# GradientSpaces/LivingScenes

Measured on AMD Instinct MI355X. Metric: object-instances/sec (encode+match+register), N=1024 pts, higher is better.
Workload: dtype f32 (GEMM products as two-piece f16 splits on the f16 matrix cores, fp32 accumulate: as accurate against fp64 as an fp32 FMA chain)

## Files before the change

### livingscenes_amd/csrc/edge_fused.hip

```cpp
#include "ls_common.h"

namespace ls {

constexpr int FK = 16;
constexpr int FND = 32;
typedef _Float16 fh8_t __attribute__((ext_vector_type(8)));
typedef _Float16 fh2_t __attribute__((ext_vector_type(2)));
typedef float ff2_t __attribute__((ext_vector_type(2)));
typedef float ff16_t __attribute__((ext_vector_type(16)));

__device__ __forceinline__ void fsplit_pair(ff2_t v, unsigned& h, unsigned& l) {
    const fh2_t hv = __builtin_convertvector(v, fh2_t);
    const fh2_t lv = __builtin_convertvector(v - __builtin_convertvector(hv, ff2_t), fh2_t);
    h = __builtin_bit_cast(unsigned, hv);
    l = __builtin_bit_cast(unsigned, lv);
}
__device__ __forceinline__ void fpow2(float amax, float& s, int& e_inv) {
    unsigned be = (__float_as_uint(amax) >> 23) & 0xffu;
    be = be < 15u ? 15u : be;
    s = __uint_as_float((268u - be) << 23);
    e_inv = (int)be - 14 - 127;
}
template <int CTRL>
__device__ __forceinline__ float fdpp_max(float v) {
    return fmaxf(v, __int_as_float(__builtin_amdgcn_update_dpp(__float_as_int(v), __float_as_int(v), CTRL, 0xF, 0xF, false)));
}
template <int CTRL>
__device__ __forceinline__ float fdpp_add(float v) {
    return v + __int_as_float(__builtin_amdgcn_update_dpp(0, __float_as_int(v), CTRL, 0xF, 0xF, true));
}
__device__ __forceinline__ float fquad_sum(float v) { return fdpp_add<0x4E>(fdpp_add<0xB1>(v)); }
__device__ __forceinline__ float fquad_max(float v) { return fdpp_max<0x4E>(fdpp_max<0xB1>(v)); }
__device__ __forceinline__ float finv_fro(float ss) { return __builtin_amdgcn_rsqf(fmaxf(ss, 1e-24f)); }

__global__ __launch_bounds__(64) void edge_ft_presplit_w_kernel(const float* __restrict__ W, int Co, int Cin, int KS, uint4* __restrict__ planes,
                                                                int* __restrict__ wexp) {
    const int T = blockIdx.x / KS, ks = blockIdx.x % KS, lane = threadIdx.x;
    const int head = T / 5, p = T % 5, r = lane & 31;
    const float* wr = W + ((size_t)(2 * p + (r >> 4)) * Co + 16 * head + (r & 15)) * Cin;
    float am = 0.f;
    for (int c = 0; c < Cin; ++c) am = fmaxf(am, fabsf(wr[c]));
    float sc;
    int e;
    fpow2(am, sc, e);
    if (ks == 0 && lane < 32) wexp[T * 32 + r] = e;
    const int k = ks * 16 + 8 * (lane >> 5);
    uint4 h, l;
    fsplit_pair(ff2_t{wr[k] * sc, wr[k + 1] * sc}, h.x, l.x);
    fsplit_pair(ff2_t{wr[k + 2] * sc, wr[k + 3] * sc}, h.y, l.y);
    fsplit_pair(ff2_t{wr[k + 4] * sc, wr[k + 5] * sc}, h.z, l.z);
    fsplit_pair(ff2_t{wr[k + 6] * sc, wr[k + 7] * sc}, h.w, l.w);
    planes[((size_t)blockIdx.x * 2) * 64 + lane] = h;
    planes[((size_t)blockIdx.x * 2 + 1) * 64 + lane] = l;
}
size_t edge_ft_w_bytes(int Co, int Cin) { return (size_t)(Co / 16) * 5 * (Cin / 16) * 2 * 64 * sizeof(uint4) + (size_t)(Co / 16) * 5 * 32 * sizeof(int); }
int edge_ft_presplit_w_launch(const float* W, int Co, int Cin, void* planes, hipStream_t st) {
    const int tiles = (Co / 16) * 5, KS = Cin / 16;
    hipLaunchKernelGGL(edge_ft_presplit_w_kernel, dim3(tiles * KS), dim3(64), 0, st, W, Co, Cin, KS, (uint4*)planes,
                       (int*)((uint4*)planes + (size_t)tiles * KS * 128));
    LS_LAUNCH_CHECK();
    return LS_OK;
}

template <int KS>
__global__ __launch_bounds__(256) void edge_ft_prep_a_kernel(const float* __restrict__ cur, const int32_t* __restrict__ rows, int Ns, int Nd,
                                                             uint4* __restrict__ planes, int* __restrict__ aexp) {
    constexpr int CIN = KS * 16, KPW = KS / 4;
    __shared__ float lmax[4][32];
    const int lane = threadIdx.x & 63, w = threadIdx.x >> 6, j = lane & 31, h = lane >> 5;
    const int R = blockIdx.x * 32 + j;
    size_t src = (size_t)R;
    if (rows) {
        const int x = R % 3, pn = R / 3, b = pn / Nd;
        src = ((size_t)b * Ns + rows[pn]) * 3 + x;
    }
    const float* rp = cur + src * CIN + (w * KPW) * 16 + h * 8;
    float4 v[KPW][2];
    float am = 0.f;
#pragma unroll
    for (int kk = 0; kk < KPW; ++kk) {
        v[kk][0] = *reinterpret_cast<const float4*>(rp + kk * 16);
        v[kk][1] = *reinterpret_cast<const float4*>(rp + kk * 16 + 4);
    }
#pragma unroll
    for (int kk = 0; kk < KPW; ++kk)
#pragma unroll
        for (int u = 0; u < 2; ++u)
            am = fmaxf(am, fmaxf(fmaxf(fabsf(v[kk][u].x), fabsf(v[kk][u].y)), fmaxf(fabsf(v[kk][u].z), fabsf(v[kk][u].w))));
    am = fmaxf(am, __shfl_xor(am, 32, 64));
    if (h == 0) lmax[w][j] = am;
    __syncthreads();
    am = fmaxf(fmaxf(lmax[0][j], lmax[1][j]), fmaxf(lmax[2][j], lmax[3][j]));
    float sc;
    int e;
    fpow2(am, sc, e);
    if (w == 0 && h == 0) aexp[R] = e;
#pragma unroll
    for (int kk = 0; kk < KPW; ++kk) {
        uint4 hh, ll;
        fsplit_pair(ff2_t{v[kk][0].x * sc, v[kk][0].y * sc}, hh.x, ll.x);
        fsplit_pair(ff2_t{v[kk][0].z * sc, v[kk][0].w * sc}, hh.y, ll.y);
        fsplit_pair(ff2_t{v[kk][1].x * sc, v[kk][1].y * sc}, hh.z, ll.z);
        fsplit_pair(ff2_t{v[kk][1].z * sc, v[kk][1].w * sc}, hh.w, ll.w);
        uint4* op = planes + (((size_t)blockIdx.x * KS + w * KPW + kk) * 2) * 64 + lane;
        op[0] = hh;
        op[64] = ll;
    }
}

struct FT43 { float4 x, y, z; };
__device__ __forceinline__ FT43 ft_lds43(const float* p, int sld) {
    FT43 r;
    r.x = *reinterpret_cast<const float4*>(p);
    r.y = *reinterpret_cast<const float4*>(p + sld);
    r.z = *reinterpret_cast<const float4*>(p + 2 * sld);
    return r;
}
__device__ __forceinline__ FT43 ft_add43(const FT43& a, const FT43& b) {
    FT43 r;
    r.x = make_float4(a.x.x + b.x.x, a.x.y + b.x.y, a.x.z + b.x.z, a.x.w + b.x.w);
    r.y = make_float4(a.y.x + b.y.x, a.y.y + b.y.y, a.y.z + b.y.z, a.y.w + b.y.w);
    r.z = make_float4(a.z.x + b.z.x, a.z.y + b.z.y, a.z.z + b.z.z, a.z.w + b.z.w);
    return r;
}
__device__ __forceinline__ void ft_act43(FT43& y, const FT43& k, float oms) {
    vn_act(y.x.x, y.y.x, y.z.x, k.x.x, k.y.x, k.z.x, oms);
    vn_act(y.x.y, y.y.y, y.z.y, k.x.y, k.y.y, k.z.y, oms);
    vn_act(y.x.z, y.y.z, y.z.z, k.x.z, k.y.z, k.z.z, oms);
    vn_act(y.x.w, y.y.w, y.z.w, k.x.w, k.y.w, k.z.w, oms);
}
__device__ __forceinline__ float ft_dot43(const FT43& a, const FT43& b) {
    float s = a.x.x * b.x.x;
    s = __builtin_fmaf(a.y.x, b.y.x, s); s = __builtin_fmaf(a.z.x, b.z.x, s);
    s = __builtin_fmaf(a.x.y, b.x.y, s); s = __builtin_fmaf(a.y.y, b.y.y, s); s = __builtin_fmaf(a.z.y, b.z.y, s);
    s = __builtin_fmaf(a.x.z, b.x.z, s); s = __builtin_fmaf(a.y.z, b.y.z, s); s = __builtin_fmaf(a.z.z, b.z.z, s);
    s = __builtin_fmaf(a.x.w, b.x.w, s); s = __builtin_fmaf(a.y.w, b.y.w, s); s = __builtin_fmaf(a.z.w, b.z.w, s);
    return s;
}
__device__ __forceinline__ void ft_fma43(FT43& acc, float w, const FT43& y) {
    acc.x.x = __builtin_fmaf(w, y.x.x, acc.x.x); acc.x.y = __builtin_fmaf(w, y.x.y, acc.x.y); acc.x.z = __builtin_fmaf(w, y.x.z, acc.x.z); acc.x.w = __builtin_fmaf(w, y.x.w, acc.x.w);
    acc.y.x = __builtin_fmaf(w, y.y.x, acc.y.x); acc.y.y = __builtin_fmaf(w, y.y.y, acc.y.y); acc.y.z = __builtin_fmaf(w, y.y.z, acc.y.z); acc.y.w = __builtin_fmaf(w, y.y.w, acc.y.w);
    acc.z.x = __builtin_fmaf(w, y.z.x, acc.z.x); acc.z.y = __builtin_fmaf(w, y.z.y, acc.z.y); acc.z.z = __builtin_fmaf(w, y.z.z, acc.z.z); acc.z.w = __builtin_fmaf(w, y.z.w, acc.z.w);
}

template <int KS>
struct FtJob { const uint4* a_planes; const int* a_exp; int mt0; int MT; int p; float* slab; int sld; };

template <int KS, int MPU>
__device__ __forceinline__ void ft_gemm_unit(const FtJob<KS>& jb, int tile0, int hl, int T, const uint4* __restrict__ wplanes, const int* __restrict__ wexp, int lane) {
    const char* ab = reinterpret_cast<const char*>(jb.a_planes + ((size_t)(jb.mt0 + tile0) * KS * 2) * 64);
    const char* wb = reinterpret_cast<const char*>(wplanes + ((size_t)T * KS * 2) * 64);
    const int we = wexp[T * 32 + (lane & 31)];
    ff16_t acc[MPU];
#pragma unroll
    for (int m = 0; m < MPU; ++m)
#pragma unroll
        for (int r = 0; r < 16; ++r) acc[m][r] = 0.f;
    unsigned voff = (unsigned)lane * 16u;
    constexpr int KB = 2;
    struct Stage { fh8_t ah[MPU][KB], al[MPU][KB], bh[KB], bl[KB]; };
    auto load_stage = [&](Stage& sg, int k0) {
        asm volatile("" : "+v"(voff));
#pragma unroll
        for (int u = 0; u < KB; ++u) {
            sg.bh[u] = __builtin_bit_cast(fh8_t, *reinterpret_cast<const uint4*>(wb + (size_t)((k0 + u) * 2) * 1024 + voff));
            sg.bl[u] = __builtin_bit_cast(fh8_t, *reinterpret_cast<const uint4*>(wb + (size_t)((k0 + u) * 2 + 1) * 1024 + voff));
#pragma unroll
            for (int m = 0; m < MPU; ++m) {
                sg.ah[m][u] = __builtin_bit_cast(fh8_t, *reinterpret_cast<const uint4*>(ab + (size_t)((m * KS + k0 + u) * 2) * 1024 + voff));
                sg.al[m][u] = __builtin_bit_cast(fh8_t, *reinterpret_cast<const uint4*>(ab + (size_t)((m * KS + k0 + u) * 2 + 1) * 1024 + voff));
            }
        }
    };
    auto run_stage = [&](const Stage& sg) {
#pragma unroll
        for (int u = 0; u < KB; ++u)
#pragma unroll
            for (int m = 0; m < MPU; ++m) {
                acc[m] = __builtin_amdgcn_mfma_f32_32x32x16_f16(sg.al[m][u], sg.bh[u], acc[m], 0, 0, 0);
                acc[m] = __builtin_amdgcn_mfma_f32_32x32x16_f16(sg.ah[m][u], sg.bh[u], acc[m], 0, 0, 0);
                acc[m] = __builtin_amdgcn_mfma_f32_32x32x16_f16(sg.ah[m][u], sg.bl[u], acc[m], 0, 0, 0);
            }
#pragma unroll
        for (int m = 0; m < MPU; ++m) asm volatile("" : "+v"(acc[m])::"memory");
    };
#pragma unroll
    for (int k0 = 0; k0 < KS; k0 += KB) {
        Stage sg;
        load_stage(sg, k0);
        __builtin_amdgcn_sched_barrier(0);
        run_stage(sg);
    }
#pragma unroll
    for (int m = 0; m < MPU; ++m) {
        const int mt = tile0 + m;
        const int row0 = 32 * mt + 4 * (lane >> 5);
        float* sp = jb.slab + (size_t)row0 * jb.sld + hl * 32 + (lane & 31);
        const int* ae = jb.a_exp + (jb.mt0 + mt) * 32 + 4 * (lane >> 5);
#pragma unroll
        for (int r = 0; r < 16; ++r) {
            const int dr = (r & 3) + 8 * (r >> 2);
            sp[dr * jb.sld] = __builtin_ldexpf(acc[m][r], ae[dr] + we);
        }
    }
}
template <int KS, int HG, int NJ>
__device__ __forceinline__ void ft_gemm_phase_g3(const FtJob<KS> (&jobs)[NJ], const uint4* __restrict__ wplanes, const int* __restrict__ wexp, int head0,
                                                 int wave, int lane) {
    if constexpr (NJ == 2 && HG == 1) {
        if (jobs[0].MT == 12 && jobs[1].MT == 3) {
            ft_gemm_unit<KS, 3>(jobs[0], 3 * wave, 0, head0 * 5 + jobs[0].p, wplanes, wexp, lane);
            if (wave < 3) ft_gemm_unit<KS, 1>(jobs[1], wave, 0, head0 * 5 + jobs[1].p, wplanes, wexp, lane);
            return;
        }
    }
    int total = 0;
#pragma unroll
    for (int j = 0; j < NJ; ++j) total += (jobs[j].MT / 3) * HG;
    for (int t = wave; t < total; t += 4) {
        int j = 0, off = t;
#pragma unroll
        for (int q = 0; q < NJ - 1; ++q)
            if (j == q && off >= (jobs[q].MT / 3) * HG) { off -= (jobs[q].MT / 3) * HG; j = q + 1; }
        FtJob<KS> jb = jobs[0];
#pragma unroll
        for (int q = 1; q < NJ; ++q)
            if (j == q) jb = jobs[q];
        const int ng = jb.MT / 3, hl = off / ng, g = off - hl * ng;
        ft_gemm_unit<KS, 3>(jb, 3 * g, hl, (head0 + hl) * 5 + jb.p, wplanes, wexp, lane);
    }
}

template <int KS, int HG, int NJ>
__device__ __forceinline__ void ft_gemm_phase_shared(const FtJob<KS> (&jobs)[NJ], const uint4* __restrict__ wplanes, const int* __restrict__ wexp, int head0,
                                                     int wave, int lane, uint4* ring) {
    const bool has_unit = wave < NJ * HG;
    const int j = has_unit ? wave / HG : 0, hl = wave % HG;
    FtJob<KS> jb = jobs[0];
#pragma unroll
    for (int q = 1; q < NJ; ++q)
        if (j == q) jb = jobs[q];
    const int T = (head0 + hl) * 5 + jb.p;
    const char* ab = reinterpret_cast<const char*>(jobs[0].a_planes + ((size_t)jobs[0].mt0 * KS * 2) * 64);
    const char* wb = reinterpret_cast<const char*>(wplanes + ((size_t)T * KS * 2) * 64);
    const int we = wexp[T * 32 + (lane & 31)];
    ff16_t acc[3];
#pragma unroll
    for (int m = 0; m < 3; ++m)
#pragma unroll
        for (int r = 0; r < 16; ++r) acc[m][r] = 0.f;
    unsigned voff = (unsigned)lane * 16u;
    auto a_addr = [&](int k0, int f) { const int u = f / 6, m = (f % 6) / 2, pl = f % 2; return ab + (size_t)((m * KS + k0 + u) * 2 + pl) * 1024 + voff; };
    constexpr int NB = KS / 2;
    uint4 sA_r0, sA_r1, sA_r2, sA_w0, sA_w1, sA_w2, sA_w3, sB_r0, sB_r1, sB_r2, sB_w0, sB_w1, sB_w2, sB_w3, sC_r0, sC_r1, sC_r2, sC_w0, sC_w1, sC_w2, sC_w3;
#define LS_FT_LOAD_BATCH(S, K0)                                                                           \
    {                                                                                                     \
        asm volatile("" : "+v"(voff));                                                                    \
        S##_r0 = *reinterpret_cast<const uint4*>(a_addr((K0), wave * 3 + 0));                             \
        S##_r1 = *reinterpret_cast<const uint4*>(a_addr((K0), wave * 3 + 1));                             \
        S##_r2 = *reinterpret_cast<const uint4*>(a_addr((K0), wave * 3 + 2));                             \
        S##_w0 = *reinterpret_cast<const uint4*>(wb + (size_t)(((K0) + 0) * 2) * 1024 + voff);            \
        S##_w1 = *reinterpret_cast<const uint4*>(wb + (size_t)(((K0) + 0) * 2 + 1) * 1024 + voff);        \
        S##_w2 = *reinterpret_cast<const uint4*>(wb + (size_t)(((K0) + 1) * 2) * 1024 + voff);            \
        S##_w3 = *reinterpret_cast<const uint4*>(wb + (size_t)(((K0) + 1) * 2 + 1) * 1024 + voff);        \
    }
#define LS_FT_STEP(S, BI)                                                                                                                          \
    {                                                                                                                                              \
        uint4* rb = ring + ((BI) & 1) * 12 * 64;                                                                                                   \
        rb[(wave * 3 + 0) * 64 + lane] = S##_r0;                                                                                                   \
        rb[(wave * 3 + 1) * 64 + lane] = S##_r1;                                                                                                   \
        rb[(wave * 3 + 2) * 64 + lane] = S##_r2;                                                                                                   \
        const fh8_t bh0 = __builtin_bit_cast(fh8_t, S##_w0), bl0 = __builtin_bit_cast(fh8_t, S##_w1), bh1 = __builtin_bit_cast(fh8_t, S##_w2),     \
                    bl1 = __builtin_bit_cast(fh8_t, S##_w3);                                                                                       \
        if ((BI) + 3 < NB) LS_FT_LOAD_BATCH(S, 2 * ((BI) + 3))                                                                                     \
        __syncthreads();                                                                                                                           \
        if (has_unit) {                                                                                                                            \
            _Pragma("unroll") for (int u = 0; u < 2; ++u) {                                                                                        \
                const fh8_t bh = u ? bh1 : bh0, bl = u ? bl1 : bl0;                                                                                \
                _Pragma("unroll") for (int m = 0; m < 3; ++m) {                                                                                    \
                    const fh8_t ah = __builtin_bit_cast(fh8_t, rb[(u * 6 + m * 2) * 64 + lane]), al = __builtin_bit_cast(fh8_t, rb[(u * 6 + m * 2 + 1) * 64 + lane]); \
                    acc[m] = __builtin_amdgcn_mfma_f32_32x32x16_f16(al, bh, acc[m], 0, 0, 0);                                                      \
                    acc[m] = __builtin_amdgcn_mfma_f32_32x32x16_f16(ah, bh, acc[m], 0, 0, 0);                                                      \
                    acc[m] = __builtin_amdgcn_mfma_f32_32x32x16_f16(ah, bl, acc[m], 0, 0, 0);                                                      \
                }                                                                                                                                  \
            }                                                                                                                                      \
        }                                                                                                                                          \
    }
    LS_FT_LOAD_BATCH(sA, 0)
    if (1 < NB) LS_FT_LOAD_BATCH(sB, 2)
    if (2 < NB) LS_FT_LOAD_BATCH(sC, 4)
#pragma unroll
    for (int bi = 0; bi < NB; bi += 3) {
        LS_FT_STEP(sA, bi)
        if (bi + 1 < NB) LS_FT_STEP(sB, bi + 1)
        if (bi + 2 < NB) LS_FT_STEP(sC, bi + 2)
    }
#undef LS_FT_STEP
#undef LS_FT_LOAD_BATCH
    if (has_unit) {
#pragma unroll
        for (int m = 0; m < 3; ++m) {
            const int row0 = 32 * m + 4 * (lane >> 5);
            float* sp = jb.slab + (size_t)row0 * jb.sld + hl * 32 + (lane & 31);
            const int* ae = jb.a_exp + (jb.mt0 + m) * 32 + 4 * (lane >> 5);
#pragma unroll
            for (int r = 0; r < 16; ++r) {
                const int dr = (r & 3) + 8 * (r >> 2);
                sp[dr * jb.sld] = __builtin_ldexpf(acc[m][r], ae[dr] + we);
            }
        }
    }
}

template <int HG>
struct FtMap {
    int n, hl, ql, k0, kn;
    __device__ __forceinline__ FtMap(int tid) {
        ql = tid & 3;
        const int idx = tid >> 2;
        n = idx >> 1;
        if constexpr (HG == 2) { hl = idx & 1; k0 = 0; kn = FK; }
        else { hl = 0; k0 = (idx & 1) * (FK / 2); kn = FK / 2; }
    }
};

template <int CIN, int NS, int HG>
__global__ __launch_bounds__(256, 2) void edge_ft_qk_kernel(const uint4* __restrict__ a_p, const int* __restrict__ ae_p, const uint4* __restrict__ a_q,
                                                         const int* __restrict__ ae_q, const uint4* __restrict__ wplanes, const int* __restrict__ wexp,
                                                         const int32_t* __restrict__ knn, int B, int H, float oms, float* __restrict__ scores,
                                                         float* __restrict__ sskp, float* __restrict__ ssqp) {
    constexpr int KS = CIN / 16, MTP = NS * 3 / 32, MTQ = FND * 3 / 32, SLD = HG * 32 + 4;
    __shared__ __attribute__((aligned(16))) float slab_q[FND * 3 * SLD];
    __shared__ __attribute__((aligned(16))) float slab_p[NS * 3 * SLD];
    __shared__ __attribute__((aligned(16))) uint4 a_ring[NS == 32 ? 2 * 12 * 64 : 1];
    const int tid = threadIdx.x, lane = tid & 63, wave = __builtin_amdgcn_readfirstlane(tid >> 6);
    const int logical = xcd_remap(blockIdx.x, gridDim.x);
    const int ngroups = H / HG;
    const int hg = logical % ngroups, b = logical / ngroups, head0 = hg * HG;
    const FtMap<HG> mp(tid);
    const int head = head0 + mp.hl;

    {
        const FtJob<KS> jq[1] = {{a_q, ae_q, b * MTQ, MTQ, 4, slab_q, SLD}};
        if constexpr (NS == 32) ft_gemm_phase_shared<KS, HG, 1>(jq, wplanes, wexp, head0, wave, lane, a_ring);
        else ft_gemm_phase_g3<KS, HG, 1>(jq, wplanes, wexp, head0, wave, lane);
    }
    __syncthreads();
    const int c4 = mp.hl * 32 + mp.ql * 4;
    FT43 qf = ft_lds43(slab_q + (size_t)(3 * mp.n) * SLD + c4, SLD);
    {
        const FT43 kd = ft_lds43(slab_q + (size_t)(3 * mp.n) * SLD + c4 + 16, SLD);
        ft_act43(qf, kd, oms);
    }
    const float ssq = fquad_sum(ft_dot43(qf, qf));
    if (mp.ql == 0 && mp.k0 == 0) ssqp[((size_t)b * H + head) * FND + mp.n] = ssq;
    int nb[FK];
    {
        const int4* kp = reinterpret_cast<const int4*>(knn + ((size_t)b * FND + mp.n) * FK + mp.k0);
#pragma unroll
        for (int u = 0; u < FK / 4; ++u)
            if (4 * u < mp.kn) { const int4 v = kp[u]; nb[4 * u] = v.x; nb[4 * u + 1] = v.y; nb[4 * u + 2] = v.z; nb[4 * u + 3] = v.w; }
    }
    __syncthreads();

    {
        const FtJob<KS> jk[2] = {{a_p, ae_p, b * MTP, MTP, 1, slab_p, SLD}, {a_q, ae_q, b * MTQ, MTQ, 3, slab_q, SLD}};
        if constexpr (NS == 32) ft_gemm_phase_shared<KS, HG, 2>(jk, wplanes, wexp, head0, wave, lane, a_ring);
        else ft_gemm_phase_g3<KS, HG, 2>(jk, wplanes, wexp, head0, wave, lane);
    }
    __syncthreads();
    {
        const FT43 ql = ft_lds43(slab_q + (size_t)(3 * mp.n) * SLD + c4, SLD), qd = ft_lds43(slab_q + (size_t)(3 * mp.n) * SLD + c4 + 16, SLD);
        float* so = scores + (((size_t)b * H + head) * FND + mp.n) * FK + mp.k0;
        float* ko = sskp + (((size_t)b * H + head) * FND + mp.n) * FK + mp.k0;
#pragma unroll
        for (int k = 0; k < FK; ++k) {
            if (k < mp.kn) {
                const float* pr = slab_p + (size_t)(3 * nb[k]) * SLD + c4;
                FT43 y = ft_add43(ft_lds43(pr, SLD), ql);
                const FT43 kd = ft_add43(ft_lds43(pr + 16, SLD), qd);
                ft_act43(y, kd, oms);
                const float s2 = fquad_sum(ft_dot43(y, y));
                const float a = fquad_sum(ft_dot43(y, qf));
                if (mp.ql == 0) { so[k] = a; ko[k] = s2; }
            }
        }
    }
}

__global__ __launch_bounds__(256) void edge_ft_norms_kernel(const float* __restrict__ sskp, const float* __restrict__ ssqp, int H, float* __restrict__ invk,
                                                            float* __restrict__ invq) {
    LS_LATENCY_CRITICAL();
    const int b = blockIdx.x, tid = threadIdx.x;
    for (int e = tid; e < FND * FK + FND; e += 256) {
        const bool isk = e < FND * FK;
        const int stride = isk ? FND * FK : FND;
        const float* sp = isk ? sskp + (size_t)b * H * FND * FK + e : ssqp + (size_t)b * H * FND + (e - FND * FK);
        float s = 0.f;
        int h = 0;
        for (; h + 8 <= H; h += 8) {
            float v[8];
#pragma unroll
            for (int u = 0; u < 8; ++u) v[u] = sp[(size_t)(h + u) * stride];
#pragma unroll
            for (int u = 0; u < 8; ++u) s += v[u];
        }
        for (; h < H; ++h) s += sp[(size_t)h * stride];
        if (isk) invk[(size_t)b * FND * FK + e] = finv_fro(s);
        else invq[(size_t)b * FND + (e - FND * FK)] = finv_fro(s);
    }
}

template <int CIN, int NS, int HG>
__global__ __launch_bounds__(256, 2) void edge_ft_v_kernel(const uint4* __restrict__ a_p, const int* __restrict__ ae_p, const uint4* __restrict__ a_q,
                                                        const int* __restrict__ ae_q, const uint4* __restrict__ wplanes, const int* __restrict__ wexp,
                                                        const int32_t* __restrict__ knn, int B, int H, float oms, float inv_sqrt_dk,
                                                        const float* __restrict__ scores, const float* __restrict__ invk, const float* __restrict__ invq,
                                                        float* __restrict__ out, int Co, float* __restrict__ rowmax, int rm_parts, float* __restrict__ colsum) {
    constexpr int KS = CIN / 16, MTP = NS * 3 / 32, MTQ = FND * 3 / 32, SLD = HG * 32 + 4;
    __shared__ __attribute__((aligned(16))) float slab_q[FND * 3 * SLD];
    __shared__ __attribute__((aligned(16))) float slab_p[NS * 3 * SLD];
    __shared__ __attribute__((aligned(16))) uint4 a_ring[NS == 32 ? 2 * 12 * 64 : 1];
    const int tid = threadIdx.x, lane = tid & 63, wave = __builtin_amdgcn_readfirstlane(tid >> 6);
    const int logical = xcd_remap(blockIdx.x, gridDim.x);
    const int ngroups = H / HG;
    const int hg = logical % ngroups, b = logical / ngroups, head0 = hg * HG;
    const FtMap<HG> mp(tid);
    const int head = head0 + mp.hl;

    int nb[FK];
    float4 sraw[FK / 4], ik4[FK / 4];
    float iq;
    {
        const int4* kp = reinterpret_cast<const int4*>(knn + ((size_t)b * FND + mp.n) * FK);
        const float4* sp = reinterpret_cast<const float4*>(scores + (((size_t)b * H + head) * FND + mp.n) * FK);
        const float4* ip = reinterpret_cast<const float4*>(invk + ((size_t)b * FND + mp.n) * FK);
#pragma unroll
        for (int u = 0; u < FK / 4; ++u) {
            const int4 v = kp[u];
            nb[4 * u] = v.x; nb[4 * u + 1] = v.y; nb[4 * u + 2] = v.z; nb[4 * u + 3] = v.w;
            sraw[u] = sp[u];
            ik4[u] = ip[u];
        }
        iq = invq[(size_t)b * FND + mp.n] * inv_sqrt_dk;
    }
    {
        const FtJob<KS> jv[2] = {{a_p, ae_p, b * MTP, MTP, 0, slab_p, SLD}, {a_q, ae_q, b * MTQ, MTQ, 2, slab_q, SLD}};
        if constexpr (NS == 32) ft_gemm_phase_shared<KS, HG, 2>(jv, wplanes, wexp, head0, wave, lane, a_ring);
        else ft_gemm_phase_g3<KS, HG, 2>(jv, wplanes, wexp, head0, wave, lane);
    }
    __syncthreads();
    float wgt[FK];
    float sum = 0.f;
    {
        float mx = -INFINITY;
#pragma unroll
        for (int u = 0; u < FK / 4; ++u) {
            const float4 v = sraw[u], ik = ik4[u];
            wgt[4 * u] = v.x * iq * ik.x;
            wgt[4 * u + 1] = v.y * iq * ik.y;
            wgt[4 * u + 2] = v.z * iq * ik.z;
            wgt[4 * u + 3] = v.w * iq * ik.w;
        }
#pragma unroll
        for (int k = 0; k < FK; ++k) mx = fmaxf(mx, wgt[k]);
#pragma unroll
        for (int k = 0; k < FK; ++k) { wgt[k] = expf(wgt[k] - mx); sum += wgt[k]; }
    }
    const int c4 = mp.hl * 32 + mp.ql * 4;
    FT43 acc;
    acc.x = acc.y = acc.z = make_float4(0.f, 0.f, 0.f, 0.f);
    {
        const FT43 ql = ft_lds43(slab_q + (size_t)(3 * mp.n) * SLD + c4, SLD), qd = ft_lds43(slab_q + (size_t)(3 * mp.n) * SLD + c4 + 16, SLD);
#pragma unroll
        for (int k = 0; k < FK; ++k) {
            if (k >= mp.k0 && k < mp.k0 + mp.kn) {
                const float* pr = slab_p + (size_t)(3 * nb[k]) * SLD + c4;
                FT43 y = ft_add43(ft_lds43(pr, SLD), ql);
                const FT43 kd = ft_add43(ft_lds43(pr + 16, SLD), qd);
                ft_act43(y, kd, oms);
                ft_fma43(acc, wgt[k], y);
            }
        }
    }
    if constexpr (HG == 1) {
        auto comb = [&](float v) { const float o = __shfl_xor(v, 4, 64); return (tid & 4) ? o + v : v + o; };
        acc.x = make_float4(comb(acc.x.x), comb(acc.x.y), comb(acc.x.z), comb(acc.x.w));
        acc.y = make_float4(comb(acc.y.x), comb(acc.y.y), comb(acc.y.z), comb(acc.y.w));
        acc.z = make_float4(comb(acc.z.x), comb(acc.z.y), comb(acc.z.z), comb(acc.z.w));
    }
    const float inv = 1.0f / sum;
    const float4 ox = make_float4(acc.x.x * inv, acc.x.y * inv, acc.x.z * inv, acc.x.w * inv);
    const float4 oy = make_float4(acc.y.x * inv, acc.y.y * inv, acc.y.z * inv, acc.y.w * inv);
    const float4 oz = make_float4(acc.z.x * inv, acc.z.y * inv, acc.z.z * inv, acc.z.w * inv);
    const bool writer = HG == 2 || (tid & 4) == 0;
    if (writer) {
        float* op = out + ((size_t)b * FND + mp.n) * 3 * Co + head * 16 + mp.ql * 4;
        *reinterpret_cast<float4*>(op) = ox;
        *reinterpret_cast<float4*>(op + Co) = oy;
        *reinterpret_cast<float4*>(op + 2 * Co) = oz;
    }
    if (rowmax) {
        auto amax4 = [](const float4& v) { return fmaxf(fmaxf(fabsf(v.x), fabsf(v.y)), fmaxf(fabsf(v.z), fabsf(v.w))); };
        float rx = fquad_max(amax4(ox)), ry = fquad_max(amax4(oy)), rz = fquad_max(amax4(oz));
        if constexpr (HG == 2) {
            rx = fmaxf(rx, __shfl_xor(rx, 4, 64)); ry = fmaxf(ry, __shfl_xor(ry, 4, 64)); rz = fmaxf(rz, __shfl_xor(rz, 4, 64));
        }
        if ((tid & 7) == 0) {
            float* rp = rowmax + (((size_t)b * FND + mp.n) * 3) * rm_parts + hg;
            rp[0] = rx; rp[rm_parts] = ry; rp[2 * rm_parts] = rz;
        }
    }
    if (colsum) {
        constexpr int CW = HG * 16;
        __syncthreads();
        if (writer) {
            float* cp = slab_q + mp.n * 3 * CW + mp.hl * 16 + mp.ql * 4;
            *reinterpret_cast<float4*>(cp) = ox;
            *reinterpret_cast<float4*>(cp + CW) = oy;
            *reinterpret_cast<float4*>(cp + 2 * CW) = oz;
        }
        __syncthreads();
        if (tid < 3 * CW) {
            float a = 0.f;
#pragma unroll 8
            for (int n = 0; n < FND; ++n) a += slab_q[n * 3 * CW + tid];
            const int ax = tid / CW, c = tid - ax * CW;
            colsum[((size_t)b * 3 + ax) * Co + head0 * 16 + c] = a;
        }
    }
}

bool edge_ft_supported(int Co, int Cin, int Ns, int Nd, int head_c, bool has_rows) {
    if (head_c != 16 || Nd != FND) return false;
    if (Cin == 128 && Ns == 128 && has_rows && Co % 16 == 0) return true;
    if (Cin == 256 && Ns == 32 && !has_rows && Co % 32 == 0) return true;
    return false;
}
int edge_ft_heads_per_group(int Cin) { return Cin == 256 ? 2 : 1; }
size_t edge_ft_scratch_bytes(int B, int Ns, int Nd, int Cin, int Co, bool has_rows) {
    const size_t rp = (size_t)B * Ns * 3, rq = (size_t)B * Nd * 3, H = Co / 16;
    size_t s = rp * Cin * 4 + rp * 4 + 512;
    if (has_rows) s += rq * Cin * 4 + rq * 4 + 512;
    s += 2 * ((size_t)B * H * Nd * FK * 4 + 256) + (size_t)B * H * Nd * 4 + 256;
    s += (size_t)B * Nd * FK * 4 + 256 + (size_t)B * Nd * 4 + 256;
    return s;
}
struct FtScratch { uint4* a_p; int* ae_p; uint4* a_q; int* ae_q; float* scores; float* sskp; float* ssqp; float* invk; float* invq; };
static FtScratch ft_layout(void* scratch, int B, int Ns, int Nd, int Cin, int Co, bool has_rows) {
    auto up = [](size_t v) { return (v + 255) & ~(size_t)255; };
    const size_t rp = (size_t)B * Ns * 3, rq = (size_t)B * Nd * 3, H = Co / 16;
    char* c = (char*)scratch;
    FtScratch s;
    size_t off = 0;
    s.a_p = (uint4*)(c + off); off = up(off + rp * Cin * 4);
    s.ae_p = (int*)(c + off); off = up(off + rp * 4);
    if (has_rows) {
        s.a_q = (uint4*)(c + off); off = up(off + rq * Cin * 4);
        s.ae_q = (int*)(c + off); off = up(off + rq * 4);
    } else { s.a_q = s.a_p; s.ae_q = s.ae_p; }
    s.scores = (float*)(c + off); off = up(off + (size_t)B * H * Nd * FK * 4);
    s.sskp = (float*)(c + off); off = up(off + (size_t)B * H * Nd * FK * 4);
    s.ssqp = (float*)(c + off); off = up(off + (size_t)B * H * Nd * 4);
    s.invk = (float*)(c + off); off = up(off + (size_t)B * Nd * FK * 4);
    s.invq = (float*)(c + off);
    return s;
}
int edge_ft_prep_launch(const float* cur, const int32_t* dst_rows, int B, int Ns, int Nd, int Cin, int Co, void* scratch, hipStream_t st) {
    const bool has_rows = dst_rows != nullptr;
    LS_REQUIRE(edge_ft_supported(Co, Cin, Ns, Nd, 16, has_rows), "edge_ft_prep: unsupported shape (Co=%d Cin=%d Ns=%d Nd=%d)", Co, Cin, Ns, Nd);
    const FtScratch s = ft_layout(scratch, B, Ns, Nd, Cin, Co, has_rows);
    if (Cin == 128) {
        hipLaunchKernelGGL(edge_ft_prep_a_kernel<8>, dim3(B * Ns * 3 / 32), dim3(256), 0, st, cur, (const int32_t*)nullptr, Ns, Nd, s.a_p, s.ae_p);
        LS_LAUNCH_CHECK();
        hipLaunchKernelGGL(edge_ft_prep_a_kernel<8>, dim3(B * Nd * 3 / 32), dim3(256), 0, st, cur, dst_rows, Ns, Nd, s.a_q, s.ae_q);
    } else {
        hipLaunchKernelGGL(edge_ft_prep_a_kernel<16>, dim3(B * Ns * 3 / 32), dim3(256), 0, st, cur, (const int32_t*)nullptr, Ns, Nd, s.a_p, s.ae_p);
    }
    LS_LAUNCH_CHECK();
    return LS_OK;
}
int edge_ft_attn_launch(const void* wplanes, const int32_t* knn, bool has_rows, int B, int Ns, int Nd, int Cin, int Co, float neg_slope, void* scratch,
                        float* out, float* rowmax, hipStream_t st, float* colsum) {
    LS_REQUIRE(edge_ft_supported(Co, Cin, Ns, Nd, 16, has_rows) && wplanes, "edge_ft_attn: unsupported shape (Co=%d Cin=%d Ns=%d Nd=%d)", Co, Cin, Ns, Nd);
    const FtScratch s = ft_layout(scratch, B, Ns, Nd, Cin, Co, has_rows);
    const int H = Co / 16, HG = edge_ft_heads_per_group(Cin), KS = Cin / 16;
    const uint4* wp = (const uint4*)wplanes;
    const int* we = (const int*)(wp + (size_t)H * 5 * KS * 128);
    const float oms = 1.0f - neg_slope, isd = 1.0f / sqrtf(3.0f * 16);
    const dim3 grid((H / HG) * B);
    if (Cin == 128) {
        hipLaunchKernelGGL((edge_ft_qk_kernel<128, 128, 1>), grid, dim3(256), 0, st, s.a_p, s.ae_p, s.a_q, s.ae_q, wp, we, knn, B, H, oms, s.scores, s.sskp, s.ssqp);
        LS_LAUNCH_CHECK();
        hipLaunchKernelGGL(edge_ft_norms_kernel, dim3(B), dim3(256), 0, st, s.sskp, s.ssqp, H, s.invk, s.invq);
        LS_LAUNCH_CHECK();
        hipLaunchKernelGGL((edge_ft_v_kernel<128, 128, 1>), grid, dim3(256), 0, st, s.a_p, s.ae_p, s.a_q, s.ae_q, wp, we, knn, B, H, oms, isd, s.scores, s.invk,
                           s.invq, out, Co, rowmax, H / HG, colsum);
    } else {
        hipLaunchKernelGGL((edge_ft_qk_kernel<256, 32, 2>), grid, dim3(256), 0, st, s.a_p, s.ae_p, s.a_q, s.ae_q, wp, we, knn, B, H, oms, s.scores, s.sskp, s.ssqp);
        LS_LAUNCH_CHECK();
        hipLaunchKernelGGL(edge_ft_norms_kernel, dim3(B), dim3(256), 0, st, s.sskp, s.ssqp, H, s.invk, s.invq);
        LS_LAUNCH_CHECK();
        hipLaunchKernelGGL((edge_ft_v_kernel<256, 32, 2>), grid, dim3(256), 0, st, s.a_p, s.ae_p, s.a_q, s.ae_q, wp, we, knn, B, H, oms, isd, s.scores, s.invk,
                           s.invq, out, Co, rowmax, H / HG, colsum);
    }
    LS_LAUNCH_CHECK();
    return LS_OK;
}
int edge_ft_rowmax_parts(int Co, int Cin) { return Co / 16 / edge_ft_heads_per_group(Cin); }

}
```

Measured before the change: 56840.

## Fuse query and key projection GEMMs into one pass sharing A-fragment loads

Merges the separate Q-projection and K-projection GEMM phases into a single pass per wave. Each wave computes several weight tiles against the same A fragments, and in the 32-sample path the A tiles are shared through the LDS ring with prefetch depth as a template parameter. The K tile for the query slab is held in registers across the first attention step and written after a barrier. This removes one full GEMM pass with its barriers and repeated A loads, at the cost of more accumulator registers and templated code that is harder to follow.

```diff
diff --git a/livingscenes_amd/csrc/edge_fused.hip b/livingscenes_amd/csrc/edge_fused.hip
--- a/livingscenes_amd/csrc/edge_fused.hip
+++ b/livingscenes_amd/csrc/edge_fused.hip
@@ -143,173 +143,158 @@
     acc.z.x = __builtin_fmaf(w, y.z.x, acc.z.x); acc.z.y = __builtin_fmaf(w, y.z.y, acc.z.y); acc.z.z = __builtin_fmaf(w, y.z.z, acc.z.z); acc.z.w = __builtin_fmaf(w, y.z.w, acc.z.w);
 }
 
+template <int MT, int NW>
+struct FtGroup {
+    const char* ab;
+    const char* wb[NW > 0 ? NW : 1];
+    int on;
+    int m0, mtn;
+};
 template <int KS>
-struct FtJob { const uint4* a_planes; const int* a_exp; int mt0; int MT; int p; float* slab; int sld; };
-
-template <int KS, int MPU>
-__device__ __forceinline__ void ft_gemm_unit(const FtJob<KS>& jb, int tile0, int hl, int T, const uint4* __restrict__ wplanes, const int* __restrict__ wexp, int lane) {
-    const char* ab = reinterpret_cast<const char*>(jb.a_planes + ((size_t)(jb.mt0 + tile0) * KS * 2) * 64);
-    const char* wb = reinterpret_cast<const char*>(wplanes + ((size_t)T * KS * 2) * 64);
-    const int we = wexp[T * 32 + (lane & 31)];
-    ff16_t acc[MPU];
-#pragma unroll
-    for (int m = 0; m < MPU; ++m)
-#pragma unroll
-        for (int r = 0; r < 16; ++r) acc[m][r] = 0.f;
+__device__ __forceinline__ const char* ft_a_tile(const uint4* a_planes, int tile) { return reinterpret_cast<const char*>(a_planes + ((size_t)tile * KS * 2) * 64); }
+template <int KS>
+__device__ __forceinline__ const char* ft_w_tile(const uint4* wplanes, int T) { return reinterpret_cast<const char*>(wplanes + ((size_t)T * KS * 2) * 64); }
+
+template <int MT1, int NW1, bool RING>
+struct FtBatch {
+    fh8_t a0[RING ? 3 : 12];
+    fh8_t w0[4];
+    fh8_t a1[MT1 > 0 && !RING ? MT1 * 4 : 1];
+    fh8_t w1[NW1 > 0 ? NW1 * 4 : 1];
+};
+template <int KS>
+__device__ __forceinline__ fh8_t ft_frag(const char* base, int m, int ks, int pl, unsigned voff) {
+    return *reinterpret_cast<const fh8_t*>(base + (size_t)((m * KS + ks) * 2 + pl) * 1024 + voff);
+}
+template <int KS, bool DO_A, bool DO_W, int MT1, int NW1, bool RING>
+__device__ __forceinline__ void ft_request_batch(FtBatch<MT1, NW1, RING>& s, const FtGroup<3, 1>& g0, const FtGroup<MT1, NW1>& g1, int k0, int wave, unsigned& voff) {
+    asm volatile("" : "+v"(voff));
+    if constexpr (DO_A) {
+#pragma unroll
+        for (int i = 0; i < (RING ? 3 : 12); ++i) {
+            const int f = RING ? wave * 3 + i : i;
+            s.a0[i] = ft_frag<KS>(g0.ab, (f % 6) / 2, k0 + f / 6, f % 2, voff);
+        }
+        if constexpr (MT1 > 0 && !RING) {
+            if (g1.on) {
+#pragma unroll
+                for (int f = 0; f < MT1 * 4; ++f) s.a1[f] = ft_frag<KS>(g1.ab, (f % (2 * MT1)) / 2, k0 + f / (2 * MT1), f % 2, voff);
+            }
+        }
+    }
+    if constexpr (DO_W) {
+#pragma unroll
+        for (int i = 0; i < 4; ++i) s.w0[i] = ft_frag<KS>(g0.wb[0], 0, k0, i, voff);
+        if constexpr (MT1 > 0) {
+            if (g1.on) {
+#pragma unroll
+                for (int w = 0; w < NW1; ++w)
+#pragma unroll
+                    for (int i = 0; i < 4; ++i) s.w1[w * 4 + i] = ft_frag<KS>(g1.wb[w], 0, k0, i, voff);
+            }
+        }
+    }
+}
+__device__ __forceinline__ void ft_mfma3(ff16_t& acc, fh8_t ah, fh8_t al, fh8_t bh, fh8_t bl) {
+    acc = __builtin_amdgcn_mfma_f32_32x32x16_f16(al, bh, acc, 0, 0, 0);
+    acc = __builtin_amdgcn_mfma_f32_32x32x16_f16(ah, bh, acc, 0, 0, 0);
+    acc = __builtin_amdgcn_mfma_f32_32x32x16_f16(ah, bl, acc, 0, 0, 0);
+}
+template <int MT, int NW>
+__device__ __forceinline__ void ft_mfma_regs(ff16_t (&acc)[MT * NW], const fh8_t (&a)[MT * 4], const fh8_t (&w)[NW * 4]) {
+#pragma unroll
+    for (int u = 0; u < 2; ++u)
+#pragma unroll
+        for (int m = 0; m < MT; ++m)
+#pragma unroll
+            for (int x = 0; x < NW; ++x) ft_mfma3(acc[x * MT + m], a[u * MT * 2 + m * 2], a[u * MT * 2 + m * 2 + 1], w[x * 4 + u * 2], w[x * 4 + u * 2 + 1]);
+}
+template <int MT>
+__device__ __forceinline__ void ft_mfma_ring(ff16_t (&acc)[MT], const fh8_t* rb, int m0, int mtn, const fh8_t (&w)[4]) {
+#pragma unroll
+    for (int u = 0; u < 2; ++u)
+#pragma unroll
+        for (int m = 0; m < MT; ++m)
+            if (m == 0 || m < mtn) ft_mfma3(acc[m], rb[(u * 6 + (m0 + m) * 2) * 64], rb[(u * 6 + (m0 + m) * 2 + 1) * 64], w[u * 2], w[u * 2 + 1]);
+}
+template <int KS, int ND, bool RING, int BI, int MT1, int NW1>
+__device__ __forceinline__ void ft_gemm_steps(FtBatch<MT1, NW1, RING> (&sets)[ND > 0 ? ND : 1], const FtGroup<3, 1>& g0, ff16_t (&acc0)[3], const FtGroup<MT1, NW1>& g1,
+                                              ff16_t (&acc1)[MT1 * NW1 > 0 ? MT1 * NW1 : 1], int wave, int lane, uint4* ring, unsigned& voff) {
+    constexpr int NB = KS / 2;
+    if constexpr (BI < NB) {
+        FtBatch<MT1, NW1, RING>& s = sets[ND > 0 ? BI % ND : 0];
+        if constexpr (RING) {
+            fh8_t* rb = reinterpret_cast<fh8_t*>(ring) + (BI & 1) * 12 * 64 + lane;
+#pragma unroll
+            for (int i = 0; i < 3; ++i) rb[(wave * 3 + i) * 64] = s.a0[i];
+            constexpr bool WLATE = MT1 > 0, MORE = BI + ND < NB;
+            fh8_t wc[4];
+#pragma unroll
+            for (int i = 0; i < 4; ++i) wc[i] = s.w0[i];
+            if constexpr (MORE) ft_request_batch<KS, true, !WLATE>(s, g0, g1, 2 * (BI + ND), wave, voff);
+            __syncthreads();
+            ft_mfma_ring<3>(acc0, rb, 0, 3, wc);
+            if constexpr (MT1 > 0) {
+                static_assert(MT1 == 0 || NW1 == 1, "ring group 1: one weight tile");
+                if (g1.on) ft_mfma_ring<MT1>(acc1, rb, g1.m0, g1.mtn, s.w1);
+            }
+            if constexpr (MORE && WLATE) {
+#pragma unroll
+                for (int i = 0; i < 3; ++i) asm volatile("" : "+v"(acc0[i])::"memory");
+#pragma unroll
+                for (int i = 0; i < MT1 * NW1; ++i) asm volatile("" : "+v"(acc1[i])::"memory");
+                ft_request_batch<KS, false, true>(s, g0, g1, 2 * (BI + ND), wave, voff);
+            }
+        } else {
+            ft_request_batch<KS, true, true>(s, g0, g1, 2 * BI, wave, voff);
+            __builtin_amdgcn_sched_barrier(0);
+            ft_mfma_regs<3, 1>(acc0, s.a0, s.w0);
+            if constexpr (MT1 > 0) {
+                if (g1.on) ft_mfma_regs<MT1, NW1>(acc1, s.a1, s.w1);
+            }
+        }
+#pragma unroll
+        for (int i = 0; i < 3; ++i) asm volatile("" : "+v"(acc0[i])::"memory");
+        if constexpr (MT1 > 0) {
+#pragma unroll
+            for (int i = 0; i < MT1 * NW1; ++i) asm volatile("" : "+v"(acc1[i])::"memory");
+        }
+        ft_gemm_steps<KS, ND, RING, BI + 1>(sets, g0, acc0, g1, acc1, wave, lane, ring, voff);
+    }
+}
+template <int KS, int ND, bool RING, int MT1, int NW1>
+__device__ __forceinline__ void ft_gemm_pass(const FtGroup<3, 1>& g0, ff16_t (&acc0)[3], const FtGroup<MT1, NW1>& g1, ff16_t (&acc1)[MT1 * NW1 > 0 ? MT1 * NW1 : 1],
+                                             int wave, int lane, uint4* ring) {
+    static_assert(RING ? (ND >= 1 && ND <= 3) : ND == 0, "ring: prefetched; private streams: one batch at a time");
+    constexpr int NB = KS / 2;
+#pragma unroll
+    for (int i = 0; i < 3; ++i)
+#pragma unroll
+        for (int r = 0; r < 16; ++r) acc0[i][r] = 0.f;
+#pragma unroll
+    for (int i = 0; i < (MT1 * NW1 > 0 ? MT1 * NW1 : 1); ++i)
+#pragma unroll
+        for (int r = 0; r < 16; ++r) acc1[i][r] = 0.f;
     unsigned voff = (unsigned)lane * 16u;
-    constexpr int KB = 2;
-    struct Stage { fh8_t ah[MPU][KB], al[MPU][KB], bh[KB], bl[KB]; };
-    auto load_stage = [&](Stage& sg, int k0) {
-        asm volatile("" : "+v"(voff));
-#pragma unroll
-        for (int u = 0; u < KB; ++u) {
-            sg.bh[u] = __builtin_bit_cast(fh8_t, *reinterpret_cast<const uint4*>(wb + (size_t)((k0 + u) * 2) * 1024 + voff));
-            sg.bl[u] = __builtin_bit_cast(fh8_t, *reinterpret_cast<const uint4*>(wb + (size_t)((k0 + u) * 2 + 1) * 1024 + voff));
-#pragma unroll
-            for (int m = 0; m < MPU; ++m) {
-                sg.ah[m][u] = __builtin_bit_cast(fh8_t, *reinterpret_cast<const uint4*>(ab + (size_t)((m * KS + k0 + u) * 2) * 1024 + voff));
-                sg.al[m][u] = __builtin_bit_cast(fh8_t, *reinterpret_cast<const uint4*>(ab + (size_t)((m * KS + k0 + u) * 2 + 1) * 1024 + voff));
-            }
-        }
-    };
-    auto run_stage = [&](const Stage& sg) {
-#pragma unroll
-        for (int u = 0; u < KB; ++u)
-#pragma unroll
-            for (int m = 0; m < MPU; ++m) {
-                acc[m] = __builtin_amdgcn_mfma_f32_32x32x16_f16(sg.al[m][u], sg.bh[u], acc[m], 0, 0, 0);
-                acc[m] = __builtin_amdgcn_mfma_f32_32x32x16_f16(sg.ah[m][u], sg.bh[u], acc[m], 0, 0, 0);
-                acc[m] = __builtin_amdgcn_mfma_f32_32x32x16_f16(sg.ah[m][u], sg.bl[u], acc[m], 0, 0, 0);
-            }
-#pragma unroll
-        for (int m = 0; m < MPU; ++m) asm volatile("" : "+v"(acc[m])::"memory");
-    };
-#pragma unroll
-    for (int k0 = 0; k0 < KS; k0 += KB) {
-        Stage sg;
-        load_stage(sg, k0);
-        __builtin_amdgcn_sched_barrier(0);
-        run_stage(sg);
-    }
-#pragma unroll
-    for (int m = 0; m < MPU; ++m) {
-        const int mt = tile0 + m;
-        const int row0 = 32 * mt + 4 * (lane >> 5);
-        float* sp = jb.slab + (size_t)row0 * jb.sld + hl * 32 + (lane & 31);
-        const int* ae = jb.a_exp + (jb.mt0 + mt) * 32 + 4 * (lane >> 5);
-#pragma unroll
-        for (int r = 0; r < 16; ++r) {
-            const int dr = (r & 3) + 8 * (r >> 2);
-            sp[dr * jb.sld] = __builtin_ldexpf(acc[m][r], ae[dr] + we);
-        }
-    }
-}
-template <int KS, int HG, int NJ>
-__device__ __forceinline__ void ft_gemm_phase_g3(const FtJob<KS> (&jobs)[NJ], const uint4* __restrict__ wplanes, const int* __restrict__ wexp, int head0,
-                                                 int wave, int lane) {
-    if constexpr (NJ == 2 && HG == 1) {
-        if (jobs[0].MT == 12 && jobs[1].MT == 3) {
-            ft_gemm_unit<KS, 3>(jobs[0], 3 * wave, 0, head0 * 5 + jobs[0].p, wplanes, wexp, lane);
-            if (wave < 3) ft_gemm_unit<KS, 1>(jobs[1], wave, 0, head0 * 5 + jobs[1].p, wplanes, wexp, lane);
-            return;
-        }
-    }
-    int total = 0;
-#pragma unroll
-    for (int j = 0; j < NJ; ++j) total += (jobs[j].MT / 3) * HG;
-    for (int t = wave; t < total; t += 4) {
-        int j = 0, off = t;
-#pragma unroll
-        for (int q = 0; q < NJ - 1; ++q)
-            if (j == q && off >= (jobs[q].MT / 3) * HG) { off -= (jobs[q].MT / 3) * HG; j = q + 1; }
-        FtJob<KS> jb = jobs[0];
-#pragma unroll
-        for (int q = 1; q < NJ; ++q)
-            if (j == q) jb = jobs[q];
-        const int ng = jb.MT / 3, hl = off / ng, g = off - hl * ng;
-        ft_gemm_unit<KS, 3>(jb, 3 * g, hl, (head0 + hl) * 5 + jb.p, wplanes, wexp, lane);
-    }
-}
-
-template <int KS, int HG, int NJ>
-__device__ __forceinline__ void ft_gemm_phase_shared(const FtJob<KS> (&jobs)[NJ], const uint4* __restrict__ wplanes, const int* __restrict__ wexp, int head0,
-                                                     int wave, int lane, uint4* ring) {
-    const bool has_unit = wave < NJ * HG;
-    const int j = has_unit ? wave / HG : 0, hl = wave % HG;
-    FtJob<KS> jb = jobs[0];
-#pragma unroll
-    for (int q = 1; q < NJ; ++q)
-        if (j == q) jb = jobs[q];
-    const int T = (head0 + hl) * 5 + jb.p;
-    const char* ab = reinterpret_cast<const char*>(jobs[0].a_planes + ((size_t)jobs[0].mt0 * KS * 2) * 64);
-    const char* wb = reinterpret_cast<const char*>(wplanes + ((size_t)T * KS * 2) * 64);
-    const int we = wexp[T * 32 + (lane & 31)];
-    ff16_t acc[3];
-#pragma unroll
-    for (int m = 0; m < 3; ++m)
-#pragma unroll
-        for (int r = 0; r < 16; ++r) acc[m][r] = 0.f;
-    unsigned voff = (unsigned)lane * 16u;
-    auto a_addr = [&](int k0, int f) { const int u = f / 6, m = (f % 6) / 2, pl = f % 2; return ab + (size_t)((m * KS + k0 + u) * 2 + pl) * 1024 + voff; };
-    constexpr int NB = KS / 2;
-    uint4 sA_r0, sA_r1, sA_r2, sA_w0, sA_w1, sA_w2, sA_w3, sB_r0, sB_r1, sB_r2, sB_w0, sB_w1, sB_w2, sB_w3, sC_r0, sC_r1, sC_r2, sC_w0, sC_w1, sC_w2, sC_w3;
-#define LS_FT_LOAD_BATCH(S, K0)                                                                           \
-    {                                                                                                     \
-        asm volatile("" : "+v"(voff));                                                                    \
-        S##_r0 = *reinterpret_cast<const uint4*>(a_addr((K0), wave * 3 + 0));                             \
-        S##_r1 = *reinterpret_cast<const uint4*>(a_addr((K0), wave * 3 + 1));                             \
-        S##_r2 = *reinterpret_cast<const uint4*>(a_addr((K0), wave * 3 + 2));                             \
-        S##_w0 = *reinterpret_cast<const uint4*>(wb + (size_t)(((K0) + 0) * 2) * 1024 + voff);            \
-        S##_w1 = *reinterpret_cast<const uint4*>(wb + (size_t)(((K0) + 0) * 2 + 1) * 1024 + voff);        \
-        S##_w2 = *reinterpret_cast<const uint4*>(wb + (size_t)(((K0) + 1) * 2) * 1024 + voff);            \
-        S##_w3 = *reinterpret_cast<const uint4*>(wb + (size_t)(((K0) + 1) * 2 + 1) * 1024 + voff);        \
-    }
-#define LS_FT_STEP(S, BI)                                                                                                                          \
-    {                                                                                                                                              \
-        uint4* rb = ring + ((BI) & 1) * 12 * 64;                                                                                                   \
-        rb[(wave * 3 + 0) * 64 + lane] = S##_r0;                                                                                                   \
-        rb[(wave * 3 + 1) * 64 + lane] = S##_r1;                                                                                                   \
-        rb[(wave * 3 + 2) * 64 + lane] = S##_r2;                                                                                                   \
-        const fh8_t bh0 = __builtin_bit_cast(fh8_t, S##_w0), bl0 = __builtin_bit_cast(fh8_t, S##_w1), bh1 = __builtin_bit_cast(fh8_t, S##_w2),     \
-                    bl1 = __builtin_bit_cast(fh8_t, S##_w3);                                                                                       \
-        if ((BI) + 3 < NB) LS_FT_LOAD_BATCH(S, 2 * ((BI) + 3))                                                                                     \
-        __syncthreads();                                                                                                                           \
-        if (has_unit) {                                                                                                                            \
-            _Pragma("unroll") for (int u = 0; u < 2; ++u) {                                                                                        \
-                const fh8_t bh = u ? bh1 : bh0, bl = u ? bl1 : bl0;                                                                                \
-                _Pragma("unroll") for (int m = 0; m < 3; ++m) {                                                                                    \
-                    const fh8_t ah = __builtin_bit_cast(fh8_t, rb[(u * 6 + m * 2) * 64 + lane]), al = __builtin_bit_cast(fh8_t, rb[(u * 6 + m * 2 + 1) * 64 + lane]); \
-                    acc[m] = __builtin_amdgcn_mfma_f32_32x32x16_f16(al, bh, acc[m], 0, 0, 0);                                                      \
-                    acc[m] = __builtin_amdgcn_mfma_f32_32x32x16_f16(ah, bh, acc[m], 0, 0, 0);                                                      \
-                    acc[m] = __builtin_amdgcn_mfma_f32_32x32x16_f16(ah, bl, acc[m], 0, 0, 0);                                                      \
-                }                                                                                                                                  \
-            }                                                                                                                                      \
-        }                                                                                                                                          \
-    }
-    LS_FT_LOAD_BATCH(sA, 0)
-    if (1 < NB) LS_FT_LOAD_BATCH(sB, 2)
-    if (2 < NB) LS_FT_LOAD_BATCH(sC, 4)
-#pragma unroll
-    for (int bi = 0; bi < NB; bi += 3) {
-        LS_FT_STEP(sA, bi)
-        if (bi + 1 < NB) LS_FT_STEP(sB, bi + 1)
-        if (bi + 2 < NB) LS_FT_STEP(sC, bi + 2)
-    }
-#undef LS_FT_STEP
-#undef LS_FT_LOAD_BATCH
-    if (has_unit) {
-#pragma unroll
-        for (int m = 0; m < 3; ++m) {
-            const int row0 = 32 * m + 4 * (lane >> 5);
-            float* sp = jb.slab + (size_t)row0 * jb.sld + hl * 32 + (lane & 31);
-            const int* ae = jb.a_exp + (jb.mt0 + m) * 32 + 4 * (lane >> 5);
-#pragma unroll
-            for (int r = 0; r < 16; ++r) {
-                const int dr = (r & 3) + 8 * (r >> 2);
-                sp[dr * jb.sld] = __builtin_ldexpf(acc[m][r], ae[dr] + we);
-            }
-        }
-    }
+    FtBatch<MT1, NW1, RING> sets[ND > 0 ? ND : 1];
+    if constexpr (ND > 0 && 0 < NB) ft_request_batch<KS, true, true>(sets[0], g0, g1, 0, wave, voff);
+    if constexpr (ND > 1 && 1 < NB) ft_request_batch<KS, true, true>(sets[1], g0, g1, 2, wave, voff);
+    if constexpr (ND > 2 && 2 < NB) ft_request_batch<KS, true, true>(sets[2], g0, g1, 4, wave, voff);
+    ft_gemm_steps<KS, ND, RING, 0>(sets, g0, acc0, g1, acc1, wave, lane, ring, voff);
+}
+__device__ __forceinline__ void ft_scale_tile(ff16_t& acc, const int* ae_tile, int we, int lane) {
+    const int* ae = ae_tile + 4 * (lane >> 5);
+#pragma unroll
+    for (int r = 0; r < 16; ++r) acc[r] = __builtin_ldexpf(acc[r], ae[(r & 3) + 8 * (r >> 2)] + we);
+}
+__device__ __forceinline__ void ft_put_tile(const ff16_t& acc, float* slab, int sld, int mt, int col0, int lane) {
+    float* sp = slab + (size_t)(32 * mt + 4 * (lane >> 5)) * sld + col0 + (lane & 31);
+#pragma unroll
+    for (int r = 0; r < 16; ++r) sp[((r & 3) + 8 * (r >> 2)) * sld] = acc[r];
+}
+__device__ __forceinline__ void ft_store_tile(ff16_t acc, float* slab, int sld, int mt, int col0, const int* ae_tile, int we, int lane) {
+    ft_scale_tile(acc, ae_tile, we, lane);
+    ft_put_tile(acc, slab, sld, mt, col0, lane);
 }
 
 template <int HG>
@@ -340,10 +325,40 @@
     const FtMap<HG> mp(tid);
     const int head = head0 + mp.hl;
 
-    {
-        const FtJob<KS> jq[1] = {{a_q, ae_q, b * MTQ, MTQ, 4, slab_q, SLD}};
-        if constexpr (NS == 32) ft_gemm_phase_shared<KS, HG, 1>(jq, wplanes, wexp, head0, wave, lane, a_ring);
-        else ft_gemm_phase_g3<KS, HG, 1>(jq, wplanes, wexp, head0, wave, lane);
+    constexpr int MTH = NS == 32 ? 2 : 1;
+    ff16_t qk_acc[MTH];
+    int qk_we, qk_mt0, qk_n, qk_col;
+    if constexpr (NS == 32) {
+        const int hl = wave & 1;
+        const bool first = wave < 2;
+        const int T0 = (head0 + hl) * 5 + (first ? 4 : 1), T1 = (head0 + hl) * 5 + 3;
+        const FtGroup<3, 1> g0 = {ft_a_tile<KS>(a_p, b * MTP), {ft_w_tile<KS>(wplanes, T0)}, 1, 0, 3};
+        const FtGroup<2, 1> g1 = {nullptr, {ft_w_tile<KS>(wplanes, T1)}, 1, first ? 0 : 2, first ? 2 : 1};
+        const int we0 = wexp[T0 * 32 + (lane & 31)];
+        qk_we = wexp[T1 * 32 + (lane & 31)];
+        ff16_t acc0[3];
+        ft_gemm_pass<KS, 2, true>(g0, acc0, g1, qk_acc, wave, lane, a_ring);
+#pragma unroll
+        for (int m = 0; m < 3; ++m) ft_store_tile(acc0[m], first ? slab_q : slab_p, SLD, m, hl * 32, ae_p + (b * MTP + m) * 32, we0, lane);
+        qk_mt0 = g1.m0; qk_n = g1.mtn; qk_col = hl * 32;
+#pragma unroll
+        for (int m = 0; m < MTH; ++m)
+            if (m < qk_n) ft_scale_tile(qk_acc[m], ae_q + (b * MTQ + qk_mt0 + m) * 32, qk_we, lane);
+    } else {
+        const int Tpk = head0 * 5 + 1, Tqk = head0 * 5 + 3, Tqq = head0 * 5 + 4;
+        const bool dst = wave < MTQ;
+        const FtGroup<3, 1> g0 = {ft_a_tile<KS>(a_p, b * MTP + 3 * wave), {ft_w_tile<KS>(wplanes, Tpk)}, 1, 0, 3};
+        const FtGroup<1, 2> g1 = {ft_a_tile<KS>(a_q, b * MTQ + (dst ? wave : 0)), {ft_w_tile<KS>(wplanes, Tqq), ft_w_tile<KS>(wplanes, Tqk)}, dst, 0, 1};
+        const int we_pk = wexp[Tpk * 32 + (lane & 31)], we_qq = wexp[Tqq * 32 + (lane & 31)];
+        qk_we = wexp[Tqk * 32 + (lane & 31)];
+        ff16_t acc0[3], acc1[2];
+        ft_gemm_pass<KS, 0, false>(g0, acc0, g1, acc1, wave, lane, a_ring);
+#pragma unroll
+        for (int m = 0; m < 3; ++m) ft_store_tile(acc0[m], slab_p, SLD, 3 * wave + m, 0, ae_p + (b * MTP + 3 * wave + m) * 32, we_pk, lane);
+        if (dst) ft_store_tile(acc1[0], slab_q, SLD, wave, 0, ae_q + (b * MTQ + wave) * 32, we_qq, lane);
+        qk_acc[0] = acc1[1];
+        qk_mt0 = wave; qk_n = dst ? 1 : 0; qk_col = 0;
+        if (dst) ft_scale_tile(qk_acc[0], ae_q + (b * MTQ + wave) * 32, qk_we, lane);
     }
     __syncthreads();
     const int c4 = mp.hl * 32 + mp.ql * 4;
@@ -362,12 +377,9 @@
             if (4 * u < mp.kn) { const int4 v = kp[u]; nb[4 * u] = v.x; nb[4 * u + 1] = v.y; nb[4 * u + 2] = v.z; nb[4 * u + 3] = v.w; }
     }
     __syncthreads();
-
-    {
-        const FtJob<KS> jk[2] = {{a_p, ae_p, b * MTP, MTP, 1, slab_p, SLD}, {a_q, ae_q, b * MTQ, MTQ, 3, slab_q, SLD}};
-        if constexpr (NS == 32) ft_gemm_phase_shared<KS, HG, 2>(jk, wplanes, wexp, head0, wave, lane, a_ring);
-        else ft_gemm_phase_g3<KS, HG, 2>(jk, wplanes, wexp, head0, wave, lane);
-    }
+#pragma unroll
+    for (int m = 0; m < MTH; ++m)
+        if (m < qk_n) ft_put_tile(qk_acc[m], slab_q, SLD, qk_mt0 + m, qk_col, lane);
     __syncthreads();
     {
         const FT43 ql = ft_lds43(slab_q + (size_t)(3 * mp.n) * SLD + c4, SLD), qd = ft_lds43(slab_q + (size_t)(3 * mp.n) * SLD + c4 + 16, SLD);
@@ -444,10 +456,26 @@
         }
         iq = invq[(size_t)b * FND + mp.n] * inv_sqrt_dk;
     }
-    {
-        const FtJob<KS> jv[2] = {{a_p, ae_p, b * MTP, MTP, 0, slab_p, SLD}, {a_q, ae_q, b * MTQ, MTQ, 2, slab_q, SLD}};
-        if constexpr (NS == 32) ft_gemm_phase_shared<KS, HG, 2>(jv, wplanes, wexp, head0, wave, lane, a_ring);
-        else ft_gemm_phase_g3<KS, HG, 2>(jv, wplanes, wexp, head0, wave, lane);
+    if constexpr (NS == 32) {
+        const int hl = wave & 1, T = (head0 + hl) * 5 + (wave < 2 ? 0 : 2);
+        const FtGroup<3, 1> g0 = {ft_a_tile<KS>(a_p, b * MTP), {ft_w_tile<KS>(wplanes, T)}, 1, 0, 3};
+        const FtGroup<0, 0> g1 = {nullptr, {nullptr}, 0, 0, 0};
+        const int we = wexp[T * 32 + (lane & 31)];
+        ff16_t acc[3], none[1];
+        ft_gemm_pass<KS, 3, true>(g0, acc, g1, none, wave, lane, a_ring);
+#pragma unroll
+        for (int m = 0; m < 3; ++m) ft_store_tile(acc[m], wave < 2 ? slab_p : slab_q, SLD, m, hl * 32, ae_p + (b * MTP + m) * 32, we, lane);
+    } else {
+        const int Tpv = head0 * 5, Tqv = head0 * 5 + 2;
+        const bool dst = wave < MTQ;
+        const FtGroup<3, 1> g0 = {ft_a_tile<KS>(a_p, b * MTP + 3 * wave), {ft_w_tile<KS>(wplanes, Tpv)}, 1, 0, 3};
+        const FtGroup<1, 1> g1 = {ft_a_tile<KS>(a_q, b * MTQ + (dst ? wave : 0)), {ft_w_tile<KS>(wplanes, Tqv)}, dst, 0, 1};
+        const int we_pv = wexp[Tpv * 32 + (lane & 31)], we_qv = wexp[Tqv * 32 + (lane & 31)];
+        ff16_t acc0[3], acc1[1];
+        ft_gemm_pass<KS, 0, false>(g0, acc0, g1, acc1, wave, lane, a_ring);
+#pragma unroll
+        for (int m = 0; m < 3; ++m) ft_store_tile(acc0[m], slab_p, SLD, 3 * wave + m, 0, ae_p + (b * MTP + 3 * wave + m) * 32, we_pv, lane);
+        if (dst) ft_store_tile(acc1[0], slab_q, SLD, wave, 0, ae_q + (b * MTQ + wave) * 32, we_qv, lane);
     }
     __syncthreads();
     float wgt[FK];
```

After: 57250, median of 6. Within noise of the previous version (+0.7%).
